# agakshat/spacefortress

Measured on NVIDIA B200. Metric: env-steps/sec with 84x84 obs, higher is better.
Workload: dtype f64

## Files before the change

### spacefortress_b200/csrc/sf_kernels.cu

```cuda
#include <cuda_runtime.h>
#include <stdio.h>
#include <stdlib.h>
#include <string.h>

#include <algorithm>
#include <cmath>
#include <mutex>
#include <string>
#include <vector>

#include "../../include/sf_b200.h"
#include "sf_geom.h"
#include "sf_render.cuh"
#include "sf_state.cuh"
#include "sf_step.cuh"
#include "sf_tables.h"

#define SF_BLOCK (32 * SF_RENDER_WARPS)

__host__ __device__ inline unsigned sf_hash3(unsigned seed, unsigned long long env, unsigned long long t, unsigned salt = 0x5Fu) {
  unsigned long long z = (env * 0x9E3779B97F4A7C15ull) ^ (t * 0xC2B2AE3D27D4EB4Full) ^ ((unsigned long long)seed << 32 | salt);
  z ^= z >> 30; z *= 0xBF58476D1CE4E5B9ull;
  z ^= z >> 27; z *= 0x94D049BB133111EBull;
  z ^= z >> 31;
// ... 37 lines not shown
__device__ __forceinline__ void sf_accumulate_episode(const SfDev& D, int env, SfEnv& e, bool finished, int lane) {
  int4 st0 = make_int4(0, 0, 0, 0), st1 = st0, st2 = st0;
  if (finished) { sf_flush_stats(D, env, e); st0 = __ldcg(&D.st0[env]); st1 = __ldcg(&D.st1[env]); st2 = __ldcg(&D.st2[env]); }
  sf_accumulate_episode_vals(D.epi, finished, lane, e.q3.w, e.q3.z, e.q3.x, e.q3.y, e.st3.x, st0, st1, st2);
}

__device__ __forceinline__ void sf_make_env_rec(const SfEnv& e, int env, unsigned shell_vis, SfEnvRec& r) {
  r.px = e.pos.x; r.py = e.pos.y;
  r.core = (unsigned)e.q0.x; r.pmask = (unsigned)e.q0.y;
  r.points_i = __float2int_rz(__int_as_float(e.q3.x));
  r.vuln = e.q1.z;
  r.kill_bar = (e.q1.z > 10 && e.q1.y < 250) ? 1 : 0;
  r.env = env;
  r.s0 = 0; r.ebox = 0;
  if (!(r.core & SF_CORE_SHIP_ALIVE)) {
    const SfPt c = sf_xform_base(r.px, r.py);
    r.ebox = (((c.x >> 8) - 13) + 64) | ((((c.y >> 8) - 13) + 64) << 8);
  }
  r.life = (unsigned)e.st3.z + 1u;
  r.building = 0;
  r.ns = sf_count_strokes(r.core, r.pmask, shell_vis);
  r.shell_vis = (int)shell_vis;
}

struct SfSched {
  int next_group, done;
};

struct SfRollArgs {
  int T, EB, ngroups, flags;
  const int* actions;
  unsigned action_seed;
  long long t0;
  unsigned char* obs;
  int* reward;
  unsigned char* done;
  unsigned char* fortkill;
  unsigned* events;
  SfSched* sched;
  int env0, envn;
  uint4* host_obs;
  uint4* mirror;
  unsigned long long* delta_stats;
  const unsigned char* draw_mask;
};
struct SfFeatArgs {
  float* out;
  int kind, cols;
};
struct SfStickyArgs {
  unsigned long long threshold;
  unsigned seed;
};
enum SfRollMode { SF_ROLL_STEP, SF_ROLL_STEP_HOST_DELTA, SF_ROLL_DRAW };
template <int MODE>
__device__ __forceinline__ int sf_roll_ticks(const SfRollArgs& A) { return MODE == SF_ROLL_DRAW ? 1 : A.T; }

__device__ __forceinline__ int sf_step_keys(const SfDev& D, const SfRollArgs& A, int env, int t) {
  int a = A.actions ? A.actions[(size_t)t * D.n + env]
                    : sf_hash_action(A.action_seed, (unsigned long long)(D.first_global_env + env), (unsigned long long)(A.t0 + t), D.num_actions);
  return (A.flags & SF_FLAG_ACTIONS_ARE_KEYMASKS) ? (a & 15) : D.keymask_of_action[min(max(a, 0), D.num_actions - 1)];
}
__device__ __forceinline__ void sf_store_step_out(const SfDev& D, const SfRollArgs& A, int env, int t, const SfStepOut& o) {
  size_t oi = (size_t)t * D.n + env;
  if (A.reward) A.reward[oi] = o.reward;
  if (A.done) A.done[oi] = o.done;
  if (A.fortkill) A.fortkill[oi] = o.fort_kill;
  if (A.events) A.events[oi] = o.events;
}
__device__ __forceinline__ void sf_tick_env(const SfDev& D, const SfHot* H, const SfRollArgs& A, int env, int t, bool autoreset, SfEnv& e, SfStepOut& o) {
  const int km = sf_step_keys(D, A, env, t);
  sf_env_step(D, H, env, e, km, autoreset, (A.flags & SF_FLAG_RAW_REWARD) != 0, o);
  sf_store_step_out(D, A, env, t, o);
}

__device__ __noinline__ void sf_step_group(const SfDev& D, const SfRollArgs& A, int group, int t, SfEnvRec* recs) {
  const int lane = threadIdx.x & 31;
  const SfHot* H = &sf_block_smem().hot;
  const bool autoreset = !(A.flags & SF_FLAG_NO_AUTORESET);
  const int env = A.env0 + group * A.EB + lane;
  const bool mine = lane < A.EB && env < A.env0 + A.envn;
  SfEnv e;
  bool finished = false;
  unsigned shell_vis = 0;
  SF_ST_BEGIN(__ballot_sync(0xffffffffu, mine));
  SfStepSmem& SS = sf_block_smem().step;
  const bool first_tick = t == 0, last_tick = t == A.T - 1;
  if (mine) {
    if (first_tick) sf_load_env(D, env, e);
    else {
      e.pos = SS.pos[lane]; e.vel = SS.vel[lane];
      e.q0 = SS.q0[lane]; e.q1 = SS.q1[lane]; e.q2 = SS.q2[lane]; e.q3 = SS.q3[lane]; e.st3 = SS.st3[lane];
      e.d0 = SS.d0[lane]; e.d1 = SS.d1[lane]; e.d2 = SS.d2[lane];
    }
    SF_ST_USE(e.q0.x, e.q0.y);
    SF_ST(8);
    SfStepOut o;
    sf_tick_env(D, H, A, env, t, autoreset, e, o);
    finished = o.done && autoreset;
    shell_vis = o.shell_vis;
  }
  SF_ST_RESTART(0xffffffffu);
  if (__any_sync(0xffffffffu, finished)) {
    sf_accumulate_episode(D, env, e, finished, lane);
    if (finished) { sf_new_game(D, H, env, e); shell_vis = 0; }
  }
  if (mine) {
    if (last_tick) sf_store_env(D, env, e);
    else {
      SS.pos[lane] = e.pos; SS.vel[lane] = e.vel;
      SS.q0[lane] = e.q0; SS.q1[lane] = e.q1; SS.q2[lane] = e.q2; SS.q3[lane] = e.q3; SS.st3[lane] = e.st3;
      if ((t & 7) == 7) sf_flush_stats(D, env, e);
      SS.d0[lane] = e.d0; SS.d1[lane] = e.d1; SS.d2[lane] = e.d2;
    }
    sf_make_env_rec(e, env, shell_vis, recs[lane]);
  } else recs[lane].env = -1;
  __syncwarp();
  SF_ST(15);
}

__device__ __forceinline__ void sf_load_group(const SfDev& D, const SfRollArgs& A, int group, SfEnvRec* recs) {
  const int lane = threadIdx.x & 31;
  const int env = A.env0 + group * A.EB + lane;
  const bool mine = lane < A.EB && env < A.env0 + A.envn && (!A.draw_mask || A.draw_mask[env]);
  if (mine) {
    SfEnv e;
    sf_load_env(D, env, e);
    sf_make_env_rec(e, env, sf_visible_shells(D, env, (unsigned)e.q0.y), recs[lane]);
  } else recs[lane].env = -1;
  __syncwarp();
}

template <int MODE>
__device__ __forceinline__ void sf_stepper_role(const SfDev& D, const SfRollArgs& A) {
  const int lane = threadIdx.x & 31;
  SfBlockSmem& B = sf_block_smem();
  const bool native = (A.flags & SF_FLAG_NATIVE_OBS) != 0;
  int stage = 0, group = blockIdx.x;
#pragma unroll 1
  for (int k = 0; group < A.ngroups; k = (k + 1) % SF_NEXT_GROUPS) {
    if (lane == 0) B.next_group[k] = A.sched ? (int)gridDim.x + atomicAdd(&A.sched->next_group, 1) : group + (int)gridDim.x;
    sf_stepper_ticks(D, B, lane, native, sf_roll_ticks<MODE>(A), stage, [&](int t, SfStagePrep& Tm, int h) {
      if constexpr (MODE == SF_ROLL_DRAW) sf_load_group(D, A, group, Tm.env);
      else sf_step_group(D, A, group, t, &Tm.env[32 * h]);
    });
    group = B.next_group[k];
  }
  sf_stepper_drain(stage);
  if (lane == 0 && A.sched) {
    __threadfence();
    if (atomicAdd(&A.sched->done, 1) == (int)gridDim.x - 1) { A.sched->next_group = 0; A.sched->done = 0; __threadfence(); }
  }
}
template <int MODE>
__device__ __noinline__ void sf_rollout_stepper(const SfDev& D, const SfRollArgs& A) { sf_stepper_role<MODE>(D, A); }

template <int MODE>
__device__ __forceinline__ void sf_rollout_drawer(const SfDev& D, const SfRollArgs& A) {
  const int lane = threadIdx.x & 31;
  SfBlockSmem& B = sf_block_smem();
  SfWarpSmem& W = sf_my_smem();
  SfFrameOut out;
  out.native = (A.flags & SF_FLAG_NATIVE_OBS) ? 1 : 0;
  out.obs_bytes = out.native ? (size_t)SF_NAT_H * SF_NAT_W : (size_t)84 * 84;
  out.obs = A.obs;
  out.tick_bytes = MODE == SF_ROLL_DRAW ? 0 : (size_t)D.n * out.obs_bytes;
  SfStageState st;
  st.stage = 0; st.prev_used = 0;
  int group = blockIdx.x;
#pragma unroll 1
  for (int k = 0; group < A.ngroups; k = (k + 1) % SF_NEXT_GROUPS) {
    sf_drawer_ticks(D, B, W, lane, out, sf_roll_ticks<MODE>(A), st);
    group = B.next_group[k];
  }
}

#ifndef SF_DELTA_GRANULE
#define SF_DELTA_GRANULE 64
#endif
#define SF_DELTA_LANES (SF_DELTA_GRANULE / 16)
static_assert(SF_DELTA_GRANULE == 16 || SF_DELTA_GRANULE == 32 || SF_DELTA_GRANULE == 64 || SF_DELTA_GRANULE == 128 || SF_DELTA_GRANULE == 256,
              "SF_DELTA_GRANULE must be 16, 32, 64, 128 or 256 bytes (1 to 16 lanes of a warp's ballot)");

__device__ __forceinline__ unsigned sf_host_delta_range(const uint4* cur, uint4* mirror, uint4* host, size_t c0, size_t c1, unsigned tid, unsigned nthreads) {
  const unsigned gsh = (threadIdx.x & 31) & ~(unsigned)(SF_DELTA_LANES - 1);
  unsigned sent = 0;
#pragma unroll 1
  for (size_t base = c0; base < c1; base += 4 * nthreads) {
    uint4 a[4], b[4];
#pragma unroll
    for (int u = 0; u < 4; u++) {
      const size_t i = base + u * nthreads + tid;
      a[u] = b[u] = make_uint4(0, 0, 0, 0);
      if (i < c1) { a[u] = __ldcg(cur + i); b[u] = __ldcg(mirror + i); }
    }
#pragma unroll
    for (int u = 0; u < 4; u++) {
      const size_t i = base + u * nthreads + tid;
      const bool diff = (a[u].x != b[u].x) | (a[u].y != b[u].y) | (a[u].z != b[u].z) | (a[u].w != b[u].w);
      const unsigned m = __ballot_sync(0xffffffffu, diff);
      if (m == 0) continue;
      if (i < c1 && ((m >> gsh) & ((1u << SF_DELTA_LANES) - 1u))) { host[i] = a[u]; sent++; }
      if (diff) mirror[i] = a[u];
    }
  }
  return sent;
}

__device__ __forceinline__ void sf_host_delta_count(unsigned long long* stats, unsigned sent) {
  for (int o = 16; o; o >>= 1) sent += __shfl_xor_sync(0xffffffffu, sent, o);
  if ((threadIdx.x & 31) == 0 && sent) atomicAdd(&stats[0], (unsigned long long)sent * 16u);
  if (blockIdx.x == 0 && threadIdx.x == 0) atomicAdd(&stats[1], 1ull);
}

__device__ __noinline__ void sf_block_host_delta(const SfDev& D, const SfRollArgs& A) {
  const size_t per16 = (size_t)(84 * 84) / 16;
  unsigned sent = 0;
#pragma unroll 1
  for (int group = blockIdx.x; group < A.ngroups; group += gridDim.x) {
    const int env_lo = A.env0 + group * A.EB, env_hi = min(env_lo + A.EB, A.env0 + A.envn);
    sent += sf_host_delta_range(reinterpret_cast<const uint4*>(A.obs), A.mirror, A.host_obs, (size_t)env_lo * per16, (size_t)env_hi * per16,
                                threadIdx.x, SF_BLOCK);
  }
  sf_host_delta_count(A.delta_stats, sent);
}

__global__ void __launch_bounds__(256) sf_host_delta_kernel(const uint4* __restrict__ cur, uint4* __restrict__ mirror, uint4* __restrict__ host,
                                                            size_t n16, int tail, unsigned long long* stats) {
  const unsigned sent = sf_host_delta_range(cur, mirror, host, 0, n16, blockIdx.x * blockDim.x + threadIdx.x, gridDim.x * blockDim.x);
  if (tail && blockIdx.x == 0 && threadIdx.x < (unsigned)tail) {
    const size_t o = n16 * 16 + threadIdx.x;
    const unsigned char v = reinterpret_cast<const unsigned char*>(cur)[o];
    reinterpret_cast<unsigned char*>(host)[o] = v; reinterpret_cast<unsigned char*>(mirror)[o] = v;
  }
  sf_host_delta_count(stats, sent);
}

template <int MODE>
__global__ void __launch_bounds__(SF_BLOCK, 1) sf_rollout_kernel(const __grid_constant__ SfDev D, const __grid_constant__ SfRollArgs A) {
  sf_block_smem_init(D.static_image);
  sf_warp_smem_init(sf_my_smem(), threadIdx.x & 31);
  if (threadIdx.x < 32) {
    if constexpr (MODE == SF_ROLL_DRAW) sf_stepper_role<MODE>(D, A);
    else sf_rollout_stepper<MODE>(D, A);
  } else sf_rollout_drawer<MODE>(D, A);
  if (MODE == SF_ROLL_STEP_HOST_DELTA) {
    __syncthreads();
    sf_block_host_delta(D, A);
  }
}

__global__ void __launch_bounds__(SF_BLOCK) sf_pack_static_kernel(SfDev D, unsigned char* image) {
  sf_block_smem_fill(D.tab);
  __syncthreads();
  const int4* src = reinterpret_cast<const int4*>(&sf_block_smem());
  for (int k = threadIdx.x; k < (int)(SF_STATIC_BYTES / 16); k += blockDim.x) reinterpret_cast<int4*>(image)[k] = src[k];
}

__device__ __forceinline__ void sf_forget_render_caches(const SfDev& D, int env) {
  D.expstamp[env] = 0;
  D.expo_meta[env] = make_uint2(0u, 0u);
}

__global__ void sf_seed_kernel(SfDev D, const unsigned* seeds) {
  const int env = blockIdx.x * blockDim.x + threadIdx.x;
  if (env >= D.n) return;
  SfEnv e;
  sf_load_env(D, env, e);
  sf_srand(D, env, e, seeds ? seeds[env] : 1u);
  sf_forget_render_caches(D, env);
  sf_store_env(D, env, e);
}

__global__ void sf_set_ticks_kernel(SfDev D, const int* ticks) {
  const int env = blockIdx.x * blockDim.x + threadIdx.x;
  if (env >= D.n) return;
  int4 q = D.q3[env];
  q.z = max(ticks[env], 0);
  D.q3[env] = q;
}

__global__ void sf_reset_kernel(SfDev D, const unsigned char* mask, int clear_prev_vlner) {
  const int env = blockIdx.x * blockDim.x + threadIdx.x;
  if (env >= D.n) return;
  if (mask && !mask[env]) return;
  SfEnv e;
  sf_load_env(D, env, e);
  if (clear_prev_vlner) e.q1.w = 0;
  sf_new_game(D, &D.tab->hot, env, e);
  sf_store_env(D, env, e);
}


__host__ __device__ inline int sf_feature_cols(int autoturn, int kind) { return kind == SF_OBS_MONITORS ? 10 : 15 + (autoturn ? 2 : 4); }

struct SfExtra { double vdir, aim, ndist; };
__device__ __forceinline__ SfExtra sf_compute_extra(const SfEnv& e) {
  SfExtra x;
// ... 353 lines not shown
      const unsigned pm = (unsigned)q0.y;
      D.pos[i] = *reinterpret_cast<const double2*>(rb + SF_BO_POS);
      D.vel[i] = *reinterpret_cast<const double2*>(rb + SF_BO_VEL);
      D.q0[i] = q0;
      D.q1[i] = row[SF_BO_Q / 16 + 1];
      D.q2[i] = row[SF_BO_Q / 16 + 2];
      D.q3[i] = row[SF_BO_Q / 16 + 3];
      D.st0[i] = row[SF_BO_ST / 16];
      D.st1[i] = row[SF_BO_ST / 16 + 1];
      D.st2[i] = row[SF_BO_ST / 16 + 2];
      D.st3[i] = row[SF_BO_ST / 16 + 3];
      const short* mang = reinterpret_cast<const short*>(rb + SF_BO_MANG);
#pragma unroll
      for (int s = 0; s < SF_MAX_MISSILES; s++) if ((pm >> s) & 1u) {
        D.mpos[s * np + i] = *reinterpret_cast<const double2*>(rb + SF_BO_MPOS + 16 * s);
        D.mang[s * np + i] = mang[s];
      }
#pragma unroll
      for (int s = 0; s < SF_DEV_SHELLS; s++) if ((pm >> (SF_PMASK_SHELL_SHIFT + s)) & 1u) {
        D.spos[s * np + i] = *reinterpret_cast<const double2*>(rb + SF_BO_SPOS + 16 * s);
        D.svel[s * np + i] = *reinterpret_cast<const double2*>(rb + SF_BO_SVEL + 16 * s);
        D.sang[s * np + i] = reinterpret_cast<const double*>(rb + SF_BO_SANG)[s];
      }
      const unsigned* rng = reinterpret_cast<const unsigned*>(rb + SF_BO_RNG);
#pragma unroll
      for (int w = 0; w < SF_RNG_WORDS; w++) D.rng[w * np + i] = rng[w];
      sf_forget_render_caches(D, i);
    }
    __syncwarp();
  }
}

static thread_local std::string g_err;
static int fail(int code, const std::string& msg) { g_err = msg; return code; }
#define CUDA_TRY(x) do { cudaError_t e_ = (x); if (e_ != cudaSuccess) return fail(SF_ERR_CUDA, std::string(#x) + ": " + cudaGetErrorString(e_)); } while (0)

#define SF_MAX_MIRRORS 4
#define SF_HOST_STEP_SLICES 4
struct sf_handle {
  SfDev dev;
  int device;
  int action_set;
  int gametype;
  int num_sms;
  int action_repeat;
  double sticky_p;
  SfStickyArgs sticky;
  void* slab;
  size_t slab_bytes;
  SfTables* h_tab;
  int* d_actions; unsigned char* d_obs; int* d_reward; unsigned char* d_done; unsigned char* d_kill; unsigned* d_events;
  size_t staging_obs_bytes;
  SfSched* d_sched;
  cudaStream_t host_compute, host_copy;
  cudaEvent_t host_ev[SF_HOST_STEP_SLICES];
  struct Mirror { const void* host; unsigned char* d; size_t cap, bytes; unsigned long long used; };
  Mirror mirrors[SF_MAX_MIRRORS];
  unsigned long long mirror_clock;
  unsigned long long* d_delta_stats;
  unsigned long long full_calls;

  int mirror_for(const void* host, size_t bytes, Mirror** out) {
    Mirror* mir = nullptr;
    for (auto& m : mirrors) if (m.host == host) mir = &m;
    if (!mir) {
      for (auto& m : mirrors) if (!mir || (mir->host && (!m.host || m.used < mir->used))) mir = &m;
      mir->host = nullptr;
    }
    if (bytes > mir->cap) {
      if (mir->d) { cudaFree(mir->d); mir->d = nullptr; mir->cap = 0; }
      mir->host = nullptr;
      CUDA_TRY(cudaMalloc(&mir->d, bytes));
      mir->cap = bytes;
    }
    mir->used = ++mirror_clock;
    *out = mir;
    return SF_OK;
  }
  void forget_mirrors(const void* host) {
    for (auto& m : mirrors) if (m.host == host || !host) m.host = nullptr;
  }
};

extern "C" const char* sf_last_error(void) { return g_err.c_str(); }
extern "C" int sf_version(void) { return 100; }

static int gametype_of(const char* s) {
  if (!s) return -1;
  if (!strcmp(s, "youturn")) return 0;
  if (!strcmp(s, "autoturn")) return 1;
  if (!strcmp(s, "test-youturn")) return 2;
  if (!strcmp(s, "test-autoturn")) return 3;
  return -1;
}

static int build_actions(int gametype, int action_set, int* km) {
  bool youturn = gametype == 0 || gametype == 2;
  if (action_set == 1) {
    const int tab[5] = {0, SF_KEY_FIRE, SF_KEY_THRUST, SF_KEY_LEFT, SF_KEY_RIGHT};
    int n = youturn ? 5 : 3;
    for (int i = 0; i < n; i++) km[i] = tab[i];
    return n;
  }
  if (action_set == 0 && !youturn) {
    for (int a = 0; a < 4; a++) km[a] = ((a >> 1) & 1 ? SF_KEY_FIRE : 0) | ((a & 1) ? SF_KEY_THRUST : 0);
    return 4;
  }
  if (action_set == 0 || action_set == -1) {
    for (int a = 0; a < 16; a++) {
      int m = ((a >> 1) & 1 ? SF_KEY_FIRE : 0) | ((a & 1) ? SF_KEY_THRUST : 0) | ((a >> 2) & 1 ? SF_KEY_LEFT : 0) | ((a >> 3) & 1 ? SF_KEY_RIGHT : 0);
      km[a] = youturn ? m : (m & (SF_KEY_FIRE | SF_KEY_THRUST));
    }
    return 16;
  }
  return -1;
}

template <class T>
static T* carve(char*& p, size_t count) {
  T* r = reinterpret_cast<T*>(p);
  size_t bytes = (count * sizeof(T) + 255) & ~(size_t)255;
  p += bytes;
  return r;
}

static size_t layout(SfDev& d, char* base) {
  char* p = base;
  size_t np = (size_t)d.n_pad;
  d.pos = carve<double2>(p, np); d.vel = carve<double2>(p, np);
  d.q0 = carve<int4>(p, np); d.q1 = carve<int4>(p, np); d.q2 = carve<int4>(p, np); d.q3 = carve<int4>(p, np);
  d.st0 = carve<int4>(p, np); d.st1 = carve<int4>(p, np); d.st2 = carve<int4>(p, np); d.st3 = carve<int4>(p, np);
  d.mpos = carve<double2>(p, np * SF_MAX_MISSILES); d.mang = carve<short>(p, np * SF_MAX_MISSILES);
  d.spos = carve<double2>(p, np * SF_DEV_SHELLS); d.svel = carve<double2>(p, np * SF_DEV_SHELLS); d.sang = carve<double>(p, np * SF_DEV_SHELLS);
  d.rng = carve<unsigned>(p, np * SF_RNG_WORDS);
  d.expc = carve<unsigned char>(p, np * SF_EXP_W * SF_EXP_W);
// ... 1 lines not shown
  d.expo = carve<unsigned char>(p, np * SF_EXPO_BYTES);
  d.expo_meta = carve<uint2>(p, np);
  d.epi = carve<unsigned long long>(p, SF_NUM_EPISODE_STATS);
  d.tab = carve<SfTables>(p, 1);
  d.static_image = carve<unsigned char>(p, SF_STATIC_BYTES);
  return (size_t)(p - base);
}

extern "C" int sf_destroy(sf_handle* h);

extern "C" int sf_create(const char* gametype, int action_set, int n_envs, int device, sf_handle** out) {
  if (!out) return fail(SF_ERR_INVALID, "out is NULL");
  *out = nullptr;
  int gt = gametype_of(gametype);
  if (gt < 0) return fail(SF_ERR_INVALID, std::string("cannot initialize Game. Unknown config value: `") + (gametype ? gametype : "(null)") + "'");
  if (n_envs <= 0) return fail(SF_ERR_INVALID, "n_envs must be positive");
  int km[16];
  int na = build_actions(gt, action_set, km);
  if (na < 0) return fail(SF_ERR_INVALID, "action_set must be 1, 0 or -1");
  int ndev = 0;
  CUDA_TRY(cudaGetDeviceCount(&ndev));
  if (device < 0 || device >= ndev) return fail(SF_ERR_CUDA, "no such CUDA device (this library has no CPU fallback)");
  CUDA_TRY(cudaSetDevice(device));
  int num_sms = 0;
  CUDA_TRY(cudaDeviceGetAttribute(&num_sms, cudaDevAttrMultiProcessorCount, device));

  sf_handle* h = new sf_handle();
  memset(h, 0, sizeof(*h));
  h->device = device; h->num_sms = num_sms > 0 ? num_sms : 148; h->action_set = action_set; h->gametype = gt;
  h->action_repeat = 1;
  SfDev& d = h->dev;
  d.n = n_envs; d.n_pad = (n_envs + 31) & ~31;
  d.autoturn = (gt == 1 || gt == 3);
  bool test = gt >= 2;
  d.shaped = !test;
  d.destroy_fortress = test ? 100 : 1;
  d.death_penalty = test ? 100 : 1;
  d.missile_penalty = test ? 2.0f : (float)0.05;
  d.num_actions = na;
  for (int i = 0; i < 16; i++) d.keymask_of_action[i] = i < na ? km[i] : 0;
  d.first_global_env = 0;

  h->h_tab = new SfTables();
  char err[256] = {0};
  if (sf_build_tables(h->h_tab, err, sizeof(err))) { std::string m = err; delete h->h_tab; delete h; return fail(SF_ERR_INVALID, "table build failed: " + m); }

  auto bail = [&](const char* what, cudaError_t ce) { std::string m = std::string(what) + ": " + cudaGetErrorString(ce); sf_destroy(h); return fail(SF_ERR_CUDA, m); };
  cudaError_t ce;
  h->slab_bytes = layout(d, nullptr);
  if ((ce = cudaMalloc(&h->slab, h->slab_bytes)) != cudaSuccess) return bail("cudaMalloc state slab", ce);
  layout(d, (char*)h->slab);
  if ((ce = cudaMalloc(&h->d_sched, sizeof(SfSched))) != cudaSuccess) return bail("cudaMalloc scheduler state", ce);
  if ((ce = cudaMemset(h->d_sched, 0, sizeof(SfSched))) != cudaSuccess) return bail("cudaMemset scheduler state", ce);
  if ((ce = cudaMemset(h->slab, 0, h->slab_bytes)) != cudaSuccess) return bail("cudaMemset state slab", ce);
  if ((ce = cudaMemcpy((void*)d.tab, h->h_tab, sizeof(SfTables), cudaMemcpyHostToDevice)) != cudaSuccess) return bail("upload tables", ce);
  if ((ce = cudaFuncSetAttribute(sf_rollout_kernel<SF_ROLL_STEP>, cudaFuncAttributeMaxDynamicSharedMemorySize, (int)SF_RENDER_SMEM_BYTES(SF_RENDER_WARPS))) != cudaSuccess) return bail("shared memory opt-in (rollout)", ce);
  if ((ce = cudaFuncSetAttribute(sf_rollout_kernel<SF_ROLL_STEP_HOST_DELTA>, cudaFuncAttributeMaxDynamicSharedMemorySize, (int)SF_RENDER_SMEM_BYTES(SF_RENDER_WARPS))) != cudaSuccess) return bail("shared memory opt-in (rollout, host delta)", ce);
  if ((ce = cudaFuncSetAttribute(sf_rollout_kernel<SF_ROLL_DRAW>, cudaFuncAttributeMaxDynamicSharedMemorySize, (int)SF_RENDER_SMEM_BYTES(SF_RENDER_WARPS))) != cudaSuccess) return bail("shared memory opt-in (rollout, draw)", ce);
  if ((ce = cudaFuncSetAttribute(sf_pack_static_kernel, cudaFuncAttributeMaxDynamicSharedMemorySize, (int)SF_RENDER_SMEM_BYTES(SF_RENDER_WARPS))) != cudaSuccess) return bail("shared memory opt-in (pack)", ce);
  if ((ce = cudaFuncSetAttribute(sf_save_envs_kernel, cudaFuncAttributePreferredSharedMemoryCarveout, (int)cudaSharedmemCarveoutMaxShared)) != cudaSuccess) return bail("shared memory carveout (save envs)", ce);
  if ((ce = cudaFuncSetAttribute(sf_load_envs_kernel, cudaFuncAttributePreferredSharedMemoryCarveout, (int)cudaSharedmemCarveoutMaxShared)) != cudaSuccess) return bail("shared memory carveout (load envs)", ce);
  sf_pack_static_kernel<<<1, SF_BLOCK, SF_RENDER_SMEM_BYTES(SF_RENDER_WARPS)>>>(d, const_cast<unsigned char*>(d.static_image));
  if ((ce = cudaGetLastError()) != cudaSuccess) return bail("static image kernel launch", ce);
  sf_seed_kernel<<<(d.n + 127) / 128, 128>>>(d, nullptr);
  if ((ce = cudaGetLastError()) != cudaSuccess) return bail("seed kernel launch", ce);
  if ((ce = cudaDeviceSynchronize()) != cudaSuccess) return bail("seed kernel", ce);
  *out = h;
  return SF_OK;
}

extern "C" int sf_destroy(sf_handle* h) {
  if (!h) return SF_OK;
  cudaSetDevice(h->device);
  if (h->slab) cudaFree(h->slab);
  if (h->d_actions) cudaFree(h->d_actions);
  if (h->d_obs) cudaFree(h->d_obs);
  if (h->d_reward) cudaFree(h->d_reward);
  if (h->d_done) cudaFree(h->d_done);
  if (h->d_kill) cudaFree(h->d_kill);
  if (h->d_events) cudaFree(h->d_events);
  if (h->d_sched) cudaFree(h->d_sched);
  for (auto& m : h->mirrors) if (m.d) cudaFree(m.d);
  if (h->d_delta_stats) cudaFree(h->d_delta_stats);
  if (h->host_compute) cudaStreamDestroy(h->host_compute);
  if (h->host_copy) cudaStreamDestroy(h->host_copy);
  for (int k = 0; k < SF_HOST_STEP_SLICES; k++) if (h->host_ev[k]) cudaEventDestroy(h->host_ev[k]);
  delete h->h_tab;
  delete h;
  return SF_OK;
}

extern "C" int sf_num_envs(const sf_handle* h) { return h ? h->dev.n : -1; }
extern "C" int sf_num_actions(const sf_handle* h) { return h ? h->dev.num_actions : -1; }
extern "C" int sf_action_keymask(const sf_handle* h, int action) {
  if (!h || action < 0 || action >= h->dev.num_actions) return -1;
  return h->dev.keymask_of_action[action];
}
extern "C" long long sf_state_bytes(const sf_handle* h) { return h ? (long long)h->slab_bytes : -1; }

extern "C" int sf_seed(sf_handle* h, const uint32_t* h_seeds, long long first_global_env, void* stream) {
  if (!h) return fail(SF_ERR_INVALID, "handle is NULL");
  CUDA_TRY(cudaSetDevice(h->device));
  cudaStream_t st = (cudaStream_t)stream;
  h->dev.first_global_env = first_global_env;
  unsigned* d_seeds = nullptr;
  cudaError_t ce = cudaSuccess;
  if (h_seeds) {
    CUDA_TRY(cudaMalloc(&d_seeds, sizeof(unsigned) * h->dev.n));
    ce = cudaMemcpyAsync(d_seeds, h_seeds, sizeof(unsigned) * h->dev.n, cudaMemcpyHostToDevice, st);
  }
  if (ce == cudaSuccess) {
    sf_seed_kernel<<<(h->dev.n + 127) / 128, 128, 0, st>>>(h->dev, d_seeds);
    ce = cudaGetLastError();
  }
  if (d_seeds) {
    cudaError_t cs = cudaStreamSynchronize(st);
    if (ce == cudaSuccess) ce = cs;
    cudaFree(d_seeds);
  }
  if (ce != cudaSuccess) return fail(SF_ERR_CUDA, std::string("sf_seed: ") + cudaGetErrorString(ce));
  return SF_OK;
}

static void group_shape(const sf_handle* h, int n, int* EB, int* ngroups, int* blocks) {
  const int sms = h->num_sms;
  const int eb = n <= sms * SF_GROUP_ENVS ? (n + sms - 1) / sms : SF_GROUP_ENVS;
  *EB = eb;
  *ngroups = (n + eb - 1) / eb;
  *blocks = std::min(*ngroups, sms);
}

static bool repeat_route(const sf_handle* h) { return h->action_repeat > 1 || h->sticky.threshold > 0; }

static int launch_rollout(sf_handle* h, SfRollArgs a, cudaStream_t st, bool draw = false, SfFeatArgs f = {}) {
  const SfDev& d = h->dev;
  bool render = (a.flags & SF_FLAG_RENDER) && a.obs;
  if (!draw && repeat_route(h)) {
    const int blocks = (a.envn + SF_STEP_ONLY_BLOCK - 1) / SF_STEP_ONLY_BLOCK;
    SfRollArgs s = a;
    s.flags &= ~SF_FLAG_RENDER; s.obs = nullptr; s.host_obs = nullptr; s.mirror = nullptr; s.delta_stats = nullptr;
    if (render) s.T = 1;
    const size_t n = (size_t)d.n, per = (a.flags & SF_FLAG_NATIVE_OBS) ? (size_t)SF_NAT_H * SF_NAT_W : (size_t)84 * 84;
    for (int t = 0; t < (render ? a.T : 1); t++) {
      if (render) {
        const size_t o = (size_t)t * n;
        s.actions = a.actions ? a.actions + o : nullptr; s.t0 = a.t0 + t;
        s.reward = a.reward ? a.reward + o : nullptr; s.done = a.done ? a.done + o : nullptr;
        s.fortkill = a.fortkill ? a.fortkill + o : nullptr; s.events = a.events ? a.events + o : nullptr;
      }
      const int k = h->action_repeat;
      const SfStickyArgs& y = h->sticky;
      if (y.threshold) {
        if (f.out) sf_step_repeat_kernel<true, true><<<blocks, SF_STEP_ONLY_BLOCK, 0, st>>>(d, s, f, k, y);
        else sf_step_repeat_kernel<false, true><<<blocks, SF_STEP_ONLY_BLOCK, 0, st>>>(d, s, f, k, y);
      } else {
        if (f.out) sf_step_repeat_kernel<true, false><<<blocks, SF_STEP_ONLY_BLOCK, 0, st>>>(d, s, f, k, y);
        else sf_step_repeat_kernel<false, false><<<blocks, SF_STEP_ONLY_BLOCK, 0, st>>>(d, s, f, k, y);
      }
      CUDA_TRY(cudaGetLastError());
      if (render) {
        SfRollArgs r = {};
        r.T = 1; r.obs = a.obs + (size_t)t * n * per; r.flags = a.flags; r.env0 = a.env0; r.envn = a.envn;
        if (int rc = launch_rollout(h, r, st, true)) return rc;
      }
    }
    return SF_OK;
  }
  if (render) {
    int blocks;
    group_shape(h, a.envn, &a.EB, &a.ngroups, &blocks);
    a.sched = (!draw && a.env0 == 0 && a.envn == d.n && !a.host_obs) ? h->d_sched : nullptr;
    if (draw) sf_rollout_kernel<SF_ROLL_DRAW><<<blocks, SF_BLOCK, SF_RENDER_SMEM_BYTES(SF_RENDER_WARPS), st>>>(d, a);
    else if (a.host_obs) sf_rollout_kernel<SF_ROLL_STEP_HOST_DELTA><<<blocks, SF_BLOCK, SF_RENDER_SMEM_BYTES(SF_RENDER_WARPS), st>>>(d, a);
    else sf_rollout_kernel<SF_ROLL_STEP><<<blocks, SF_BLOCK, SF_RENDER_SMEM_BYTES(SF_RENDER_WARPS), st>>>(d, a);
  } else {
    const int blocks = (a.envn + SF_STEP_ONLY_BLOCK - 1) / SF_STEP_ONLY_BLOCK;
    if (f.out) sf_step_only_kernel<true><<<blocks, SF_STEP_ONLY_BLOCK, 0, st>>>(d, a, f);
    else sf_step_only_kernel<false><<<blocks, SF_STEP_ONLY_BLOCK, 0, st>>>(d, a, f);
  }
  CUDA_TRY(cudaGetLastError());
  return SF_OK;
}

#include <cuda_bf16.h>
#define SF_PI_THREADS 192
template <bool F32>
__global__ void __launch_bounds__(SF_PI_THREADS) sf_policy_input_kernel(const unsigned char* __restrict__ frames, long long fstride, int n, const int* __restrict__ valid,
                                                                       uint4* __restrict__ out) {
  __shared__ unsigned tile[2][4 * 4 * 21];
  __shared__ unsigned lut[256];
  const int env = blockIdx.x, tid = threadIdx.x;
  for (int v = tid; v < 256; v += SF_PI_THREADS) {
    if (F32) lut[v] = __float_as_uint(__fmul_rn((float)v, __fdiv_rn(1.0f, 255.0f)));
    else { const __nv_bfloat16 h = __float2bfloat16_rn(__fdiv_rn((float)v, 255.0f)); lut[v] = *reinterpret_cast<const unsigned short*>(&h); }
  }
  const int nvalid = min(max(valid[env], 0), 4);
  const unsigned char* base = frames + (long long)env * (84 * 84);
  const int k1 = tid + SF_PI_THREADS;
  const int f0 = tid / 84, r0 = tid - f0 * 84, f1 = k1 / 84, r1 = k1 - f1 * 84;
  const bool on0 = f0 >= 4 - nvalid, on1 = k1 < 336 && f1 >= 4 - nvalid;
  const unsigned char* p0 = base + (long long)f0 * fstride + (r0 / 21) * 84 + (r0 % 21) * 4;
  const unsigned char* p1 = base + (long long)(k1 < 336 ? f1 : 0) * fstride + (r1 / 21) * 84 + (r1 % 21) * 4;
  const int X = tid >> 3, c8 = tid & 7, f = c8 >> 1, dy0 = (c8 & 1) * 2;
  const int ta = (f * 4 + dy0) * 21 + X, tb = ta + 21;
  uint4* orow = out + (long long)env * (21 * 21 * 8) * (F32 ? 2 : 1);
  auto cvt2 = [&](unsigned lo, unsigned hi) { return lut[lo] | (lut[hi] << 16); };
#pragma unroll 1
  for (int Y = 0; Y < 21; Y++) {
    unsigned* T = tile[Y & 1];
    T[tid] = on0 ? *reinterpret_cast<const unsigned*>(p0 + Y * (4 * 84)) : 0u;
    if (k1 < 336) T[k1] = on1 ? *reinterpret_cast<const unsigned*>(p1 + Y * (4 * 84)) : 0u;
    __syncthreads();
    if (tid < 21 * 8) {
      const unsigned a = T[ta], b = T[tb];
      if (F32) {
        uint4 o0, o1;
        o0.x = lut[a & 255u]; o0.y = lut[(a >> 8) & 255u]; o0.z = lut[(a >> 16) & 255u]; o0.w = lut[a >> 24];
        o1.x = lut[b & 255u]; o1.y = lut[(b >> 8) & 255u]; o1.z = lut[(b >> 16) & 255u]; o1.w = lut[b >> 24];
        orow[(Y * (21 * 8) + tid) * 2] = o0; orow[(Y * (21 * 8) + tid) * 2 + 1] = o1;
      } else {
        uint4 o;
        o.x = cvt2(a & 255u, (a >> 8) & 255u); o.y = cvt2((a >> 16) & 255u, a >> 24);
        o.z = cvt2(b & 255u, (b >> 8) & 255u); o.w = cvt2((b >> 16) & 255u, b >> 24);
        orow[Y * (21 * 8) + tid] = o;
      }
    }
  }
// ... 400 lines not shown
```

### spacefortress_b200/csrc/sf_probe.cuh

```cuda
#pragma once
#include <cuda_runtime.h>

#include "../../include/sf_b200.h"

#ifdef SF_BARRIER_TIMING
__device__ unsigned long long sf_bar_cycles[16];
__device__ __forceinline__ void sf_bar_add(int k, long long t0) { if ((threadIdx.x & 31) == 0) atomicAdd(&sf_bar_cycles[k], (unsigned long long)(clock64() - t0)); }
#define SF_BT_BEGIN() long long tb_ = clock64()
#define SF_BT(k) do { sf_bar_add(k, tb_); tb_ = clock64(); } while (0)
#define SF_ST_BEGIN(mask) unsigned stmask_ = (mask); long long ts_ = clock64()
#define SF_ST(k) do { __syncwarp(stmask_); sf_bar_add(k, ts_); ts_ = clock64(); } while (0)
#define SF_ST_RESTART(mask) do { stmask_ = (mask); ts_ = clock64(); } while (0)
#define SF_ST_USE(x, y) do { if ((x) == 0x7fffffff) (y) = 0; } while (0)

extern "C" int sf_barrier_cycles(unsigned long long* h_out, int reset) {
  cudaDeviceSynchronize();
  cudaMemcpyFromSymbol(h_out, sf_bar_cycles, sizeof(unsigned long long) * 16);
  if (reset) { unsigned long long z[16] = {0}; cudaMemcpyToSymbol(sf_bar_cycles, z, sizeof(z)); }
  return SF_OK;
}
#else
#define SF_BT_BEGIN() ((void)0)
#define SF_BT(k) ((void)0)
#define SF_ST_BEGIN(mask) ((void)0)
#define SF_ST(k) ((void)0)
#define SF_ST_RESTART(mask) ((void)0)
#define SF_ST_USE(x, y) ((void)0)
#endif

#ifdef SF_TIMELINE
#define SF_TL_BLOCKS 160
#define SF_TL_MAX 96
__device__ unsigned long long sf_tl[SF_TL_BLOCKS * 2 * SF_TL_MAX];
__device__ int sf_tl_n[SF_TL_BLOCKS * 2];
__device__ __forceinline__ void sf_tl_mark(int tag, bool first) {
  const int warp = threadIdx.x >> 5;
  if ((threadIdx.x & 31) == 0 && warp < 2 && blockIdx.x < SF_TL_BLOCKS) {
    const int i = blockIdx.x * 2 + warp;
    const int k = first ? 0 : sf_tl_n[i];
    sf_tl_n[i] = k + 1;
    if (k < SF_TL_MAX) {
      unsigned long long g;
      asm volatile("mov.u64 %0, %%globaltimer;" : "=l"(g));
      sf_tl[i * SF_TL_MAX + k] = (g << 8) | (unsigned long long)tag;
    }
  }
}
#define SF_TL_START() sf_tl_mark(1, true)
#define SF_TL(tag) sf_tl_mark(tag, false)

extern "C" int sf_timeline(unsigned long long* h_out) {
  cudaDeviceSynchronize();
  cudaMemcpyFromSymbol(h_out, sf_tl, sizeof(unsigned long long) * SF_TL_BLOCKS * 2 * SF_TL_MAX);
  static unsigned long long z[SF_TL_BLOCKS * 2 * SF_TL_MAX];
  cudaMemcpyToSymbol(sf_tl, z, sizeof(z));
  return SF_TL_MAX;
}
#else
#define SF_TL_START() ((void)0)
#define SF_TL(tag) ((void)0)
#endif
```

### spacefortress_b200/csrc/sf_render.cuh

```cuda
#pragma once
#include "sf_geom.h"
#include "sf_probe.cuh"
#include "sf_state.cuh"
#include "sf_tables.h"

#define SF_BATCH_QUADS 32
#define SF_MAX_GROUPS 256
#define SF_PATCH_STRIDE 32
#define SF_PATCH_BYTES (36 * 32)
#define SF_WIN_MAX_W 31
#define SF_WIN_MAX_H 34
#define SF_YBIAS 4096
#define SF_TAG_SHIP 0
#define SF_TAG_PROJECTILE 1
#define SF_SPAN_NONE 0xFFFFFFFFu
#define SF_QF_IRREGULAR 2

#define SF_RENDER_WARPS 24
#define SF_FORT_LIST_SMEM 48
#define SF_GROUP_ENVS 32
#define SF_STAGE_TICKS 2
#define SF_STAGE_SLOTS (SF_GROUP_ENVS * SF_STAGE_TICKS)
#define SF_ROUND_STROKES (8 * (SF_RENDER_WARPS - 1))
#define SF_CELLS_SHIP 144
// ... 1113 lines not shown
    for (int t = wi; t < (r1 - r0) * 12; t += nw) sf_phase_native_tile(D, B, W, lane, r0 + t / 12, t % 12, out, sg);
  }
  return used;
}


__device__ __forceinline__ int sf_stepper_claim(int stage) {
  const int sg = stage % SF_PREP_SLOTS;
  SF_TL(4);
  if (stage >= SF_PREP_SLOTS) sf_stage_empty_wait(sg);
  SF_TL(5);
  return sg;
}
__device__ __forceinline__ void sf_stepper_drain(int stage) {
#pragma unroll 1
  for (int s = max(stage - SF_PREP_SLOTS, 0); s < stage; s++)
    asm volatile("bar.sync %0, %1;" :: "r"(3 + SF_PREP_SLOTS + s % SF_PREP_SLOTS), "r"(32 * SF_RENDER_WARPS) : "memory");
}

template <class Prep>
__device__ __forceinline__ void sf_stepper_ticks(const SfDev& D, SfBlockSmem& B, int lane, bool native, int T, int& stage, Prep prep) {
  SfFrameOut out;
  out.obs = nullptr; out.obs_bytes = 0; out.tick_bytes = 0; out.native = native ? 1 : 0;
  int sg = sf_stepper_claim(stage);
  sf_prepare_first_round(D, B, sg, lane, 0, T, out, prep);
  SF_TL(3);
  int t = 0;
#pragma unroll 1
  for (;;) {
    sf_stage_full_arrive(sg);
    stage++;
    const SfStagePrep& Tm = B.prep[sg];
    const bool more = Tm.more != 0;
    const int nticks = Tm.nticks;
    if (!more && t + nticks >= T) break;
    const int nx = sf_stepper_claim(stage);
    SfStagePrep& Nx = B.prep[nx];
    if (more) {
#pragma unroll
      for (int h = 0; h < SF_STAGE_TICKS; h++) Nx.env[32 * h + lane] = Tm.env[32 * h + lane];
      if (lane == 0) Nx.nticks = nticks;
      __syncwarp();
      sf_round_scan(Nx, lane, Tm.r1, SF_GROUP_ENVS * nticks);
      sf_gather_strokes(D, Nx, lane, nticks - 1);
    } else {
      sf_prepare_first_round(D, B, nx, lane, t + nticks, T - (t + nticks), out, prep);
      t += nticks;
    }
    sg = nx;
  }
  SF_TL(7);
}

__device__ __forceinline__ void sf_drawer_ticks(const SfDev& D, SfBlockSmem& B, SfWarpSmem& W, int lane, SfFrameOut out, int T, SfStageState& st) {
  unsigned char* const obs0 = out.obs;
  int t = 0;
#pragma unroll 1
  for (;;) {
    const int sg = st.stage;
    SF_TL(4);
    sf_stage_full_wait(sg);
    SF_TL(5);
    const SfStagePrep& Tm = B.prep[sg];
    const bool more = Tm.more != 0;
    const int nticks = Tm.nticks;
    const bool last = !more && t + nticks >= T;
    {
      const int nz = (st.prev_used + 1) >> 1;
      for (int k = threadIdx.x - 32; k < nz; k += 32 * (SF_RENDER_WARPS - 1)) reinterpret_cast<unsigned*>(B.pool.cells)[k] = 0u;
      if (threadIdx.x == 32) B.pool.next_task = 0;
    }
    out.obs = obs0 + (size_t)t * out.tick_bytes;
    st.prev_used = sf_draw_stage(D, B, W, lane, out, sg);
    sf_stage_empty_arrive(sg);
    st.stage = sg + 1 == SF_PREP_SLOTS ? 0 : sg + 1;
    if (!more) t += nticks;
    if (last) break;
  }
  SF_TL(7);
}
```

Before: 157.5 million.

## Chain consecutive rollout launches with PDL and per-group ready queues

Consecutive STEP rollout launches now overlap through programmatic dependent launch. Each launch pushes a finished group id into a device ready queue tagged with an epoch, and the next launch's stepper warps pull group ids from that queue, spinning with acquire loads, instead of waiting for the whole previous grid to finish. This targets the tail and launch bubbles between back-to-back kernel calls. In exchange it adds spin-waits, host bookkeeping of queue counters, a sentinel stage to end the drawer loop, and the risk of deadlock or ordering bugs when launches interleave. The timeline probe is also extended to record per-launch data.

Result: faster. 159.4 million (median of 6 runs) (+1.3%).

```diff
diff --git a/spacefortress_b200/csrc/sf_kernels.cu b/spacefortress_b200/csrc/sf_kernels.cu
--- a/spacefortress_b200/csrc/sf_kernels.cu
+++ b/spacefortress_b200/csrc/sf_kernels.cu
@@ -113,6 +113,17 @@
   unsigned long long threshold;
   unsigned seed;
 };
+#ifndef SF_CHAIN_LAUNCHES
+#define SF_CHAIN_LAUNCHES 1
+#endif
+struct SfChainArgs {
+  unsigned long long* take_q;
+  unsigned* take_cnt;
+  unsigned take_base, epoch;
+  unsigned long long* push_q;
+  unsigned* push_cnt;
+  unsigned push_base, pad;
+};
 enum SfRollMode { SF_ROLL_STEP, SF_ROLL_STEP_HOST_DELTA, SF_ROLL_DRAW };
 template <int MODE>
 __device__ __forceinline__ int sf_roll_ticks(const SfRollArgs& A) { return MODE == SF_ROLL_DRAW ? 1 : A.T; }
@@ -192,20 +203,47 @@
   __syncwarp();
 }
 
+__device__ __noinline__ int sf_chain_take(const SfChainArgs& C, int ngroups) {
+  int g = ngroups;
+  if ((threadIdx.x & 31) == 0) {
+    const unsigned i = atomicAdd(C.take_cnt, 1u) - C.take_base;
+    if (i < (unsigned)ngroups) {
+      unsigned long long v;
+      for (;;) {
+        asm volatile("ld.acquire.gpu.global.u64 %0, [%1];" : "=l"(v) : "l"(C.take_q + i) : "memory");
+        if ((unsigned)(v >> 32) == C.epoch) break;
+        __nanosleep(128);
+      }
+      g = (int)(unsigned)v;
+    }
+  }
+  return __shfl_sync(0xffffffffu, g, 0);
+}
+
 template <int MODE>
-__device__ __forceinline__ void sf_stepper_role(const SfDev& D, const SfRollArgs& A) {
+__device__ __forceinline__ void sf_stepper_role(const SfDev& D, const SfRollArgs& A, const SfChainArgs& C) {
   const int lane = threadIdx.x & 31;
   SfBlockSmem& B = sf_block_smem();
   const bool native = (A.flags & SF_FLAG_NATIVE_OBS) != 0;
-  int stage = 0, group = blockIdx.x;
+  const bool chained = MODE == SF_ROLL_STEP && C.take_q;
+  int stage = 0, group = chained ? sf_chain_take(C, A.ngroups) : blockIdx.x;
 #pragma unroll 1
   for (int k = 0; group < A.ngroups; k = (k + 1) % SF_NEXT_GROUPS) {
-    if (lane == 0) B.next_group[k] = A.sched ? (int)gridDim.x + atomicAdd(&A.sched->next_group, 1) : group + (int)gridDim.x;
+    if (lane == 0) B.next_group[k] = group;
+    int next = 0;
+    if (!chained && lane == 0) next = A.sched ? (int)gridDim.x + atomicAdd(&A.sched->next_group, 1) : group + (int)gridDim.x;
     sf_stepper_ticks(D, B, lane, native, sf_roll_ticks<MODE>(A), stage, [&](int t, SfStagePrep& Tm, int h) {
       if constexpr (MODE == SF_ROLL_DRAW) sf_load_group(D, A, group, Tm.env);
       else sf_step_group(D, A, group, t, &Tm.env[32 * h]);
     });
-    group = B.next_group[k];
+    group = chained ? sf_chain_take(C, A.ngroups) : __shfl_sync(0xffffffffu, next, 0);
+  }
+  {
+    const int sg = sf_stepper_claim(stage);
+    if (lane == 0) B.prep[sg].nticks = 0;
+    __syncwarp();
+    sf_stage_full_arrive(sg);
+    stage++;
   }
   sf_stepper_drain(stage);
   if (lane == 0 && A.sched) {
@@ -214,10 +252,10 @@
   }
 }
 template <int MODE>
-__device__ __noinline__ void sf_rollout_stepper(const SfDev& D, const SfRollArgs& A) { sf_stepper_role<MODE>(D, A); }
+__device__ __noinline__ void sf_rollout_stepper(const SfDev& D, const SfRollArgs& A, const SfChainArgs& C) { sf_stepper_role<MODE>(D, A, C); }
 
 template <int MODE>
-__device__ __forceinline__ void sf_rollout_drawer(const SfDev& D, const SfRollArgs& A) {
+__device__ __forceinline__ void sf_rollout_drawer(const SfDev& D, const SfRollArgs& A, const SfChainArgs& C) {
   const int lane = threadIdx.x & 31;
   SfBlockSmem& B = sf_block_smem();
   SfWarpSmem& W = sf_my_smem();
@@ -228,11 +266,17 @@
   out.tick_bytes = MODE == SF_ROLL_DRAW ? 0 : (size_t)D.n * out.obs_bytes;
   SfStageState st;
   st.stage = 0; st.prev_used = 0;
-  int group = blockIdx.x;
 #pragma unroll 1
-  for (int k = 0; group < A.ngroups; k = (k + 1) % SF_NEXT_GROUPS) {
-    sf_drawer_ticks(D, B, W, lane, out, sf_roll_ticks<MODE>(A), st);
-    group = B.next_group[k];
+  for (int k = 0; sf_drawer_ticks(D, B, W, lane, out, sf_roll_ticks<MODE>(A), st); k = (k + 1) % SF_NEXT_GROUPS) {
+    if (MODE == SF_ROLL_STEP && C.push_q) {
+      asm volatile("fence.proxy.async.global;" ::: "memory");
+      sf_render_sync();
+      if (threadIdx.x == 32) {
+        const unsigned i = atomicAdd(C.push_cnt, 1u) - C.push_base;
+        const unsigned long long v = (unsigned long long)(C.epoch + 1u) << 32 | (unsigned)B.next_group[k];
+        asm volatile("st.release.gpu.global.u64 [%0], %1;" :: "l"(C.push_q + i), "l"(v) : "memory");
+      }
+    }
   }
 }
 
@@ -298,13 +342,15 @@
 }
 
 template <int MODE>
-__global__ void __launch_bounds__(SF_BLOCK, 1) sf_rollout_kernel(const __grid_constant__ SfDev D, const __grid_constant__ SfRollArgs A) {
+__global__ void __launch_bounds__(SF_BLOCK, 1) sf_rollout_kernel(const __grid_constant__ SfDev D, const __grid_constant__ SfRollArgs A,
+                                                                 const __grid_constant__ SfChainArgs C) {
+  if (MODE == SF_ROLL_STEP && C.push_q) asm volatile("griddepcontrol.launch_dependents;" ::: "memory");
   sf_block_smem_init(D.static_image);
   sf_warp_smem_init(sf_my_smem(), threadIdx.x & 31);
   if (threadIdx.x < 32) {
-    if constexpr (MODE == SF_ROLL_DRAW) sf_stepper_role<MODE>(D, A);
-    else sf_rollout_stepper<MODE>(D, A);
-  } else sf_rollout_drawer<MODE>(D, A);
+    if constexpr (MODE == SF_ROLL_DRAW) sf_stepper_role<MODE>(D, A, C);
+    else sf_rollout_stepper<MODE>(D, A, C);
+  } else sf_rollout_drawer<MODE>(D, A, C);
   if (MODE == SF_ROLL_STEP_HOST_DELTA) {
     __syncthreads();
     sf_block_host_delta(D, A);
@@ -764,6 +810,13 @@
   int* d_actions; unsigned char* d_obs; int* d_reward; unsigned char* d_done; unsigned char* d_kill; unsigned* d_events;
   size_t staging_obs_bytes;
   SfSched* d_sched;
+  unsigned long long* d_chain_q;
+  unsigned* d_chain_cnt;
+  int chain_depth, chain_groups;
+  unsigned chain_epoch;
+  std::vector<unsigned> chain_taken, chain_pushed;
+  cudaStream_t chain_stream;
+  bool chain_open;
   cudaStream_t host_compute, host_copy;
   cudaEvent_t host_ev[SF_HOST_STEP_SLICES];
   struct Mirror { const void* host; unsigned char* d; size_t cap, bytes; unsigned long long used; };
@@ -793,6 +846,8 @@
     for (auto& m : mirrors) if (m.host == host || !host) m.host = nullptr;
   }
 };
+
+static void group_shape(const sf_handle* h, int n, int* EB, int* ngroups, int* blocks);
 
 extern "C" const char* sf_last_error(void) { return g_err.c_str(); }
 extern "C" int sf_version(void) { return 100; }
@@ -900,6 +955,17 @@
   layout(d, (char*)h->slab);
   if ((ce = cudaMalloc(&h->d_sched, sizeof(SfSched))) != cudaSuccess) return bail("cudaMalloc scheduler state", ce);
   if ((ce = cudaMemset(h->d_sched, 0, sizeof(SfSched))) != cudaSuccess) return bail("cudaMemset scheduler state", ce);
+  {
+    int eb, blocks;
+    group_shape(h, d.n, &eb, &h->chain_groups, &blocks);
+    h->chain_depth = h->num_sms + 2;
+    const size_t qn = (size_t)h->chain_depth * h->chain_groups;
+    if ((ce = cudaMalloc(&h->d_chain_q, qn * 8)) != cudaSuccess) return bail("cudaMalloc ready queues", ce);
+    if ((ce = cudaMemset(h->d_chain_q, 0, qn * 8)) != cudaSuccess) return bail("cudaMemset ready queues", ce);
+    if ((ce = cudaMalloc(&h->d_chain_cnt, 2 * h->chain_depth * sizeof(unsigned))) != cudaSuccess) return bail("cudaMalloc queue counters", ce);
+    if ((ce = cudaMemset(h->d_chain_cnt, 0, 2 * h->chain_depth * sizeof(unsigned))) != cudaSuccess) return bail("cudaMemset queue counters", ce);
+    h->chain_taken.assign(h->chain_depth, 0u); h->chain_pushed.assign(h->chain_depth, 0u);
+  }
   if ((ce = cudaMemset(h->slab, 0, h->slab_bytes)) != cudaSuccess) return bail("cudaMemset state slab", ce);
   if ((ce = cudaMemcpy((void*)d.tab, h->h_tab, sizeof(SfTables), cudaMemcpyHostToDevice)) != cudaSuccess) return bail("upload tables", ce);
   if ((ce = cudaFuncSetAttribute(sf_rollout_kernel<SF_ROLL_STEP>, cudaFuncAttributeMaxDynamicSharedMemorySize, (int)SF_RENDER_SMEM_BYTES(SF_RENDER_WARPS))) != cudaSuccess) return bail("shared memory opt-in (rollout)", ce);
@@ -928,6 +994,8 @@
   if (h->d_kill) cudaFree(h->d_kill);
   if (h->d_events) cudaFree(h->d_events);
   if (h->d_sched) cudaFree(h->d_sched);
+  if (h->d_chain_q) cudaFree(h->d_chain_q);
+  if (h->d_chain_cnt) cudaFree(h->d_chain_cnt);
   for (auto& m : h->mirrors) if (m.d) cudaFree(m.d);
   if (h->d_delta_stats) cudaFree(h->d_delta_stats);
   if (h->host_compute) cudaStreamDestroy(h->host_compute);
@@ -983,6 +1051,7 @@
 static int launch_rollout(sf_handle* h, SfRollArgs a, cudaStream_t st, bool draw = false, SfFeatArgs f = {}) {
   const SfDev& d = h->dev;
   bool render = (a.flags & SF_FLAG_RENDER) && a.obs;
+  h->chain_open = false;
   if (!draw && repeat_route(h)) {
     const int blocks = (a.envn + SF_STEP_ONLY_BLOCK - 1) / SF_STEP_ONLY_BLOCK;
     SfRollArgs s = a;
@@ -1018,9 +1087,42 @@
     int blocks;
     group_shape(h, a.envn, &a.EB, &a.ngroups, &blocks);
     a.sched = (!draw && a.env0 == 0 && a.envn == d.n && !a.host_obs) ? h->d_sched : nullptr;
-    if (draw) sf_rollout_kernel<SF_ROLL_DRAW><<<blocks, SF_BLOCK, SF_RENDER_SMEM_BYTES(SF_RENDER_WARPS), st>>>(d, a);
-    else if (a.host_obs) sf_rollout_kernel<SF_ROLL_STEP_HOST_DELTA><<<blocks, SF_BLOCK, SF_RENDER_SMEM_BYTES(SF_RENDER_WARPS), st>>>(d, a);
-    else sf_rollout_kernel<SF_ROLL_STEP><<<blocks, SF_BLOCK, SF_RENDER_SMEM_BYTES(SF_RENDER_WARPS), st>>>(d, a);
+    SfChainArgs c = {};
+    bool chained = false;
+    if (a.sched && SF_CHAIN_LAUNCHES) {
+      cudaStreamCaptureStatus cs = cudaStreamCaptureStatusNone;
+      CUDA_TRY(cudaStreamIsCapturing(st, &cs));
+      if (cs == cudaStreamCaptureStatusNone) {
+        const unsigned e = h->chain_epoch + 1, D = (unsigned)h->chain_depth;
+        chained = h->chain_open && h->chain_stream == st && !a.actions;
+        if (chained) {
+          c.take_q = h->d_chain_q + (size_t)(e % D) * h->chain_groups; c.take_cnt = h->d_chain_cnt + e % D;
+          c.take_base = h->chain_taken[e % D];
+        }
+        c.epoch = e;
+        c.push_q = h->d_chain_q + (size_t)((e + 1) % D) * h->chain_groups; c.push_cnt = h->d_chain_cnt + D + (e + 1) % D;
+        c.push_base = h->chain_pushed[(e + 1) % D];
+      }
+    }
+    if (draw) sf_rollout_kernel<SF_ROLL_DRAW><<<blocks, SF_BLOCK, SF_RENDER_SMEM_BYTES(SF_RENDER_WARPS), st>>>(d, a, c);
+    else if (a.host_obs) sf_rollout_kernel<SF_ROLL_STEP_HOST_DELTA><<<blocks, SF_BLOCK, SF_RENDER_SMEM_BYTES(SF_RENDER_WARPS), st>>>(d, a, c);
+    else if (chained) {
+      cudaLaunchConfig_t cfg = {};
+      cudaLaunchAttribute at[1];
+      at[0].id = cudaLaunchAttributeProgrammaticStreamSerialization; at[0].val.programmaticStreamSerializationAllowed = 1;
+      cfg.gridDim = dim3(blocks); cfg.blockDim = dim3(SF_BLOCK); cfg.dynamicSmemBytes = SF_RENDER_SMEM_BYTES(SF_RENDER_WARPS);
+      cfg.stream = st; cfg.attrs = at; cfg.numAttrs = 1;
+      CUDA_TRY(cudaLaunchKernelEx(&cfg, sf_rollout_kernel<SF_ROLL_STEP>, d, a, c));
+    } else sf_rollout_kernel<SF_ROLL_STEP><<<blocks, SF_BLOCK, SF_RENDER_SMEM_BYTES(SF_RENDER_WARPS), st>>>(d, a, c);
+    CUDA_TRY(cudaGetLastError());
+    const unsigned D = (unsigned)h->chain_depth;
+    if (c.push_q) {
+      const unsigned e = c.epoch;
+      if (chained) h->chain_taken[e % D] += (unsigned)(h->chain_groups + blocks);
+      h->chain_pushed[(e + 1) % D] += (unsigned)h->chain_groups;
+      h->chain_epoch = e; h->chain_stream = st;
+    }
+    h->chain_open = c.push_q != nullptr;
   } else {
     const int blocks = (a.envn + SF_STEP_ONLY_BLOCK - 1) / SF_STEP_ONLY_BLOCK;
     if (f.out) sf_step_only_kernel<true><<<blocks, SF_STEP_ONLY_BLOCK, 0, st>>>(d, a, f);
diff --git a/spacefortress_b200/csrc/sf_probe.cuh b/spacefortress_b200/csrc/sf_probe.cuh
--- a/spacefortress_b200/csrc/sf_probe.cuh
+++ b/spacefortress_b200/csrc/sf_probe.cuh
@@ -29,21 +29,30 @@
 #endif
 
 #ifdef SF_TIMELINE
+#define SF_TL_LAUNCHES 8
 #define SF_TL_BLOCKS 160
-#define SF_TL_MAX 96
-__device__ unsigned long long sf_tl[SF_TL_BLOCKS * 2 * SF_TL_MAX];
+#define SF_TL_MAX 160
+__device__ unsigned long long sf_tl[SF_TL_LAUNCHES * SF_TL_BLOCKS * 2 * SF_TL_MAX];
 __device__ int sf_tl_n[SF_TL_BLOCKS * 2];
+__device__ int sf_tl_seq[SF_TL_BLOCKS * 2];
+__device__ __forceinline__ void sf_tl_put(int L, int i, int k, unsigned long long v) {
+  if (L < SF_TL_LAUNCHES && k < SF_TL_MAX) sf_tl[((size_t)L * SF_TL_BLOCKS * 2 + i) * SF_TL_MAX + k] = v;
+}
 __device__ __forceinline__ void sf_tl_mark(int tag, bool first) {
   const int warp = threadIdx.x >> 5;
   if ((threadIdx.x & 31) == 0 && warp < 2 && blockIdx.x < SF_TL_BLOCKS) {
     const int i = blockIdx.x * 2 + warp;
-    const int k = first ? 0 : sf_tl_n[i];
-    sf_tl_n[i] = k + 1;
-    if (k < SF_TL_MAX) {
-      unsigned long long g;
-      asm volatile("mov.u64 %0, %%globaltimer;" : "=l"(g));
-      sf_tl[i * SF_TL_MAX + k] = (g << 8) | (unsigned long long)tag;
+    if (first) { sf_tl_seq[i]++; sf_tl_n[i] = 0; }
+    const int L = sf_tl_seq[i] - 1, k = sf_tl_n[i];
+    unsigned long long g;
+    asm volatile("mov.u64 %0, %%globaltimer;" : "=l"(g));
+    sf_tl_put(L, i, k, (g << 8) | (unsigned long long)tag);
+    if (first) {
+      unsigned sm;
+      asm volatile("mov.u32 %0, %%smid;" : "=r"(sm));
+      sf_tl_put(L, i, k + 1, ((unsigned long long)sm << 8) | 6ull);
     }
+    sf_tl_n[i] = k + (first ? 2 : 1);
   }
 }
 #define SF_TL_START() sf_tl_mark(1, true)
@@ -51,9 +60,11 @@
 
 extern "C" int sf_timeline(unsigned long long* h_out) {
   cudaDeviceSynchronize();
-  cudaMemcpyFromSymbol(h_out, sf_tl, sizeof(unsigned long long) * SF_TL_BLOCKS * 2 * SF_TL_MAX);
-  static unsigned long long z[SF_TL_BLOCKS * 2 * SF_TL_MAX];
-  cudaMemcpyToSymbol(sf_tl, z, sizeof(z));
+  cudaMemcpyFromSymbol(h_out, sf_tl, sizeof(sf_tl));
+  void* p;
+  cudaGetSymbolAddress(&p, sf_tl); cudaMemset(p, 0, sizeof(sf_tl));
+  cudaGetSymbolAddress(&p, sf_tl_seq); cudaMemset(p, 0, sizeof(sf_tl_seq));
+  cudaDeviceSynchronize();
   return SF_TL_MAX;
 }
 #else
diff --git a/spacefortress_b200/csrc/sf_render.cuh b/spacefortress_b200/csrc/sf_render.cuh
--- a/spacefortress_b200/csrc/sf_render.cuh
+++ b/spacefortress_b200/csrc/sf_render.cuh
@@ -1189,7 +1189,7 @@
   SF_TL(7);
 }
 
-__device__ __forceinline__ void sf_drawer_ticks(const SfDev& D, SfBlockSmem& B, SfWarpSmem& W, int lane, SfFrameOut out, int T, SfStageState& st) {
+__device__ __forceinline__ bool sf_drawer_ticks(const SfDev& D, SfBlockSmem& B, SfWarpSmem& W, int lane, SfFrameOut out, int T, SfStageState& st) {
   unsigned char* const obs0 = out.obs;
   int t = 0;
 #pragma unroll 1
@@ -1199,8 +1199,13 @@
     sf_stage_full_wait(sg);
     SF_TL(5);
     const SfStagePrep& Tm = B.prep[sg];
+    const int nticks = Tm.nticks;
+    if (nticks == 0) {
+      sf_stage_empty_arrive(sg);
+      st.stage = sg + 1 == SF_PREP_SLOTS ? 0 : sg + 1;
+      return false;
+    }
     const bool more = Tm.more != 0;
-    const int nticks = Tm.nticks;
     const bool last = !more && t + nticks >= T;
     {
       const int nz = (st.prev_used + 1) >> 1;
@@ -1215,4 +1220,5 @@
     if (last) break;
   }
   SF_TL(7);
-}
+  return true;
+}
```
